# yukw777/EILEV

Measured on AMD Instinct MI355X. Metric: clips/sec (8-frame, 16 in-context) encode+generate, eilev-blip2-opt-2.7b, higher is better.
Workload: dtype bf16

## Files before the change

### eilev_amd/csrc/gemm_pp4.h

```cpp
#pragma once
#include "gemm_common.h"

namespace {

#ifndef EILEV_PP4_DEEP
#define EILEV_PP4_DEEP 1
#endif
template <int EPI, bool F8 = false, int LN = 0, int M16K = 0, bool A3 = false>
__global__ __launch_bounds__(512, 2) void gemm_pp4_kernel(const GemmArgs g) {
    constexpr bool M16 = M16K != 0, HT16 = M16K == 2;
    static_assert(!M16 || !F8, "16 x 16 form: bf16 instances");
    constexpr int BM = 256, BN = 256, NWM = 2, NWN = 4, NW = 8;
    constexpr int WM = BM / NWM, WN = BN / NWN, TM = WM / 32, TN = WN / 32;
    constexpr int STEP = (BM + BN) * 128;
    constexpr int PC = 8;
    static_assert(!A3 || M16, "A3: lean epilogues only");
    constexpr int STG0 = A3 ? 2 * BM * 128 : 2 * STEP;

    extern __shared__ __attribute__((aligned(16))) char smem[];
    auto a_slot = [&](int st) { return smem + (A3 ? (st % 3) * (BM * 128) : (st & 1) * STEP); };
    auto w_slot = [&](int st) { return smem + (A3 ? 3 * (BM * 128) + (st & 1) * (BN * 128) : (st & 1) * STEP + BM * 128); };
    const int tiles_m = (g.M + BM - 1) / BM, tiles_n = (g.N + BN - 1) / BN, ntiles = tiles_m * tiles_n;
    const int tid = threadIdx.x, lane = tid & 63;
    const int wid = __builtin_amdgcn_readfirstlane(tid >> 6);
// ... 169 lines not shown
            for (int i = 0; i < 4; ++i)
#pragma unroll
                for (int j = 0; j < 4; ++j)
                    acc16[i][j] = __builtin_amdgcn_mfma_f32_16x16x32_bf16(bfr[j >> 1][j & 1], af[0][i], acc16[i][j], 0, 0, 0);
        } else {
#pragma unroll
            for (int k2 = 0; k2 < 2; ++k2)
#pragma unroll
                for (int i = 0; i < 2; ++i)
#pragma unroll
                    for (int j = 0; j < 2; ++j)
                        acc[i][j] = __builtin_amdgcn_mfma_f32_32x32x16_bf16(bfr[k2][j], af[k2][i], acc[i][j], 0, 0, 0);
        }
        __builtin_amdgcn_s_setprio(0);
    };
    char *const stg = smem + STG0 + wid * 4096;
    const unsigned stg_sw = (unsigned)(STG0 + wid * 4096 + l31 * 128 + hi * 8) ^ (unsigned)((l31 & 7) << 4);
    const unsigned stg_sw16 = (unsigned)(STG0 + wid * 4096 + l15 * 128 + (g4 & 1) * 8) ^ (unsigned)((((g4 >> 1) ^ (l15 & 7)) << 4));
    const int srow = lane >> 3, schunk = lane & 7;
    auto is_lean = [&](int n0_) {
        return !(n0_ + 128 >= g.N && !(g.dbg & DBG_GEMM_NO_HALF_TILES)) && n0_ + BN <= g.N && !g.out_f32 && g.patch_group == 0 && g.scale_cols == 0 && !g.wscale && !g.ascale &&
               !(g.dbg & (DBG_GEMM_NO_EPILOGUE | DBG_GEMM_NO_STORES | DBG_GEMM_ROW0_STORES)) && !(g.dbg & DBG_GEMM_PP4_NO_PRESTAGE);
    };
    float ln_rs[LN == 1 ? (M16 ? TM16 : TM) : 1];
    auto lean_epilogue = [&](int cm0, int cn0, auto res_c, auto ht_c) {
        constexpr bool RES = decltype(res_c)::value;
        constexpr bool HTE = decltype(ht_c)::value;
        constexpr int NU = HTE ? 2 : TM;
        const int roff = HTE ? hm * 64 : wm * WM, coff = HTE ? hn * 64 : wn * WN;
        if constexpr (M16K == 1) {
            if (cn0 + coff >= g.N) return;
        }
        constexpr bool LNC = LN == 1 && !RES, LNP = LN == 2 && RES;
        typedef __attribute__((ext_vector_type(4))) unsigned u32x4_t;
        const int r0 = cm0 + roff;
        const int rows = g.M - r0 < 0 ? 0 : (g.M - r0 < NU * 32 ? g.M - r0 : NU * 32);
        auto uniform_rsrc = [&](const void *ptr, int bytes) {
            const uint64_t base = (uint64_t)ptr;
            const uint64_t ub = ((uint64_t)(unsigned)__builtin_amdgcn_readfirstlane((int)(base >> 32)) << 32) |
                                (unsigned)__builtin_amdgcn_readfirstlane((int)(unsigned)base);
            return __builtin_amdgcn_make_buffer_rsrc((void *)ub, 0, __builtin_amdgcn_readfirstlane(bytes), 0x00020000);
        };
        const __amdgpu_buffer_rsrc_t rc = uniform_rsrc(reinterpret_cast<bf16 *>(g.C) + (int64_t)r0 * g.ldc + cn0 + coff, rows * (int)(g.ldc * 2));
        const __amdgpu_buffer_rsrc_t rr = uniform_rsrc(RES ? g.resid + (int64_t)r0 * g.ldr + cn0 + coff : g.A, RES ? rows * (int)(g.ldr * 2) : 0);
        const unsigned st_voff = (unsigned)srow * (unsigned)(g.ldc * 2) + schunk * 16, rs_voff = (unsigned)srow * (unsigned)(g.ldr * 2) + schunk * 16;
#ifndef EILEV_HM_AUX
#define EILEV_HM_AUX EILEV_ST_AUX
#endif
        constexpr bool HMI = LN == 1 && !RES && EPI == 0 && M16K == 1;
        const bool hm = HMI && g.hm_tok != 0;
        __amdgpu_buffer_rsrc_t rch = rc;
        unsigned hm_off = 0, hm_off_w = 0;
        int hm_str2 = 0, hm_t = 0;
        if constexpr (HMI) {
            if (hm) {
                const int TOK = g.hm_tok, HD = g.hm_hd, NH = g.hm_heads, D3 = g.N / 3;
                const int n0 = cn0 + coff;
                const int plane = __builtin_amdgcn_readfirstlane(n0 / D3), rr = n0 - plane * D3;
                int2 ent;
                if (rr < NH * 64) {
                    ent.x = (plane * NH + (rr >> 6)) * TOK * HD + schunk * 8;
                    ent.y = 64;
                } else {
                    const int cph = (HD - 64) >> 3, jb = ((rr - NH * 64) >> 3) + schunk, hh = jb / cph;
                    ent.x = (plane * NH + hh) * TOK * HD + TOK * 64 + (jb - hh * cph) * 8;
                    ent.y = HD - 64;
                }
                const int fw = __builtin_amdgcn_readfirstlane(r0 / TOK);
                const int m0 = r0 + srow, f0 = m0 / TOK;
                hm_t = m0 - f0 * TOK;
                hm_str2 = __builtin_amdgcn_readfirstlane(ent.y * 2);
                hm_off = (unsigned)(((f0 - fw) * TOK * g.N + ent.x + hm_t * ent.y) * 2);
                hm_off_w = hm_off + (unsigned)(TOK * g.N * 2) - (unsigned)(TOK * hm_str2);
                const int64_t left = ((int64_t)g.M / TOK - fw) * TOK * g.N * 2;
                rch = uniform_rsrc(reinterpret_cast<bf16 *>(g.C) + (int64_t)fw * TOK * g.N, (int)(unsigned)(left < 0xfffffff0ll ? left : 0xfffffff0ll));
            }
        }
        u32x4_t rv[4];
        auto res_load = [&](int u) {
#pragma unroll
            for (int it = 0; it < 4; ++it) rv[it] = __builtin_amdgcn_raw_buffer_load_b128(rr, rs_voff, (u * 32 + it * 8) * (int)(g.ldr * 2), 0);
        };
        if constexpr (RES) res_load(0);
        bf16x4 biasr[M16 ? 1 : TN][4];
        bf16x4 biasr16[M16 ? TN16 : 1];
        if constexpr (M16) {
#pragma unroll
            for (int j = 0; j < TN16; ++j) {
                if (g.bias) biasr16[j] = *reinterpret_cast<const bf16x4 *>(g.bias + cn0 + coff + j * 16 + g4 * 4);
                else biasr16[j] = (bf16x4){(bf16)0.f, (bf16)0.f, (bf16)0.f, (bf16)0.f};
            }
        } else {
#pragma unroll
        for (int j = 0; j < TN; ++j)
#pragma unroll
            for (int q = 0; q < 4; ++q) {
                if (g.bias) biasr[j][q] = *reinterpret_cast<const bf16x4 *>(g.bias + cn0 + wn * WN + j * 32 + q * 8 + hi * 4);
                else biasr[j][q] = (bf16x4){(bf16)0.f, (bf16)0.f, (bf16)0.f, (bf16)0.f};
            }
        }
        typedef __attribute__((ext_vector_type(2))) float f32x2_t;
        __amdgpu_buffer_rsrc_t rst = rr;
        if constexpr (LNP) rst = uniform_rsrc(g.stat_out + ((int64_t)((cn0 + coff) >> 6) * g.stat_ld + r0) * 2, rows * 8);
        static_for<NU>([&](auto u_c) {
            constexpr int U = decltype(u_c)::value;
            float st1 = 0.0f, st2 = 0.0f;
            bf16x4 rcell[M16 ? 2 : TN][4];
            if constexpr (RES) {
#pragma unroll
                for (int it = 0; it < 4; ++it) {
                    const int row = it * 8 + srow;
                    *reinterpret_cast<u32x4_t *>(stg + row * 128 + ((schunk ^ (row & 7)) << 4)) = rv[it];
                }
                if constexpr (U + 1 < NU) res_load(U + 1);
                if constexpr (M16) {
#pragma unroll
                    for (int ib = 0; ib < 2; ++ib)
#pragma unroll
                        for (int j = 0; j < TN16; ++j) {
                            unsigned ca;
                            asm volatile("v_xor_b32 %0, %1, %2" : "=v"(ca) : "n"(((j * 2) << 4) | (ib << 11)), "v"(stg_sw16));
                            rcell[ib][j] = *reinterpret_cast<const bf16x4 *>(smem + ca);
                        }
                } else {
#pragma unroll
                for (int j = 0; j < TN; ++j)
#pragma unroll
                    for (int q = 0; q < 4; ++q) {
                        unsigned ca;
                        asm volatile("v_xor_b32 %0, %1, %2" : "=v"(ca) : "n"((j * 4 + q) << 4), "v"(stg_sw));
                        rcell[j][q] = *reinterpret_cast<const bf16x4 *>(smem + ca);
                    }
                }
            }
            float st16[2][2] = {{0.0f, 0.0f}, {0.0f, 0.0f}};
            if constexpr (M16) {
#pragma unroll
                for (int ib = 0; ib < 2; ++ib)
#pragma unroll
                    for (int j = 0; j < TN16; ++j) {
                        float v[4];
                        if constexpr (LNC) {
#pragma unroll
                            for (int e = 0; e < 4; ++e) v[e] = fmaf(acc16[2 * U + ib][j][e], ln_rs[2 * U + ib], (float)biasr16[j][e]);
                        } else {
#pragma unroll
                            for (int e = 0; e < 4; ++e) v[e] = acc16[2 * U + ib][j][e] + (float)biasr16[j][e];
                        }
                        if constexpr (LN == 0 && EPI == 0 && !RES) {
                            if (cn0 + coff + j * 16 < g.scale_cols) {
#pragma unroll
                                for (int e = 0; e < 4; ++e) v[e] *= g.scale;
                            }
                        }
                        if constexpr (EPI == 2) {
#pragma unroll
                            for (int e = 0; e < 4; ++e) v[e] = fmaxf(v[e], 0.0f);
                        }
                        if constexpr (EPI == 1) gelu_erf_n<4>(v);
                        if constexpr (RES) {
#pragma unroll
                            for (int e = 0; e < 4; ++e) v[e] += (float)rcell[ib][j][e];
                        }
                        if constexpr (LNP) {
#pragma unroll
                            for (int e = 0; e < 4; ++e) {
                                st16[ib][0] += v[e];
                                st16[ib][1] = fmaf(v[e], v[e], st16[ib][1]);
                            }
                        }
                        unsigned ca;
                        asm volatile("v_xor_b32 %0, %1, %2" : "=v"(ca) : "n"(((j * 2) << 4) | (ib << 11)), "v"(stg_sw16));
                        *reinterpret_cast<bf16x4 *>(smem + ca) = (bf16x4){(bf16)v[0], (bf16)v[1], (bf16)v[2], (bf16)v[3]};
                    }
            } else {
#pragma unroll
            for (int j = 0; j < TN; ++j)
#pragma unroll
                for (int q = 0; q < 4; ++q) {
                    float v[4];
                    if constexpr (LNC) {
#pragma unroll
                        for (int e = 0; e < 4; ++e) v[e] = fmaf(acc[U][j][q * 4 + e], ln_rs[U], (float)biasr[j][q][e]);
                    } else {
#pragma unroll
                        for (int e = 0; e < 4; ++e) v[e] = acc[U][j][q * 4 + e] + (float)biasr[j][q][e];
                    }
                    if constexpr (EPI == 2) {
#pragma unroll
                        for (int e = 0; e < 4; ++e) v[e] = fmaxf(v[e], 0.0f);
                    }
                    if constexpr (EPI == 1) gelu_erf_n<4>(v);
                    if constexpr (RES) {
#pragma unroll
                        for (int e = 0; e < 4; ++e) v[e] += (float)rcell[j][q][e];
                    }
                    if constexpr (LNP) {
#pragma unroll
                        for (int e = 0; e < 4; ++e) {
                            st1 += v[e];
                            st2 = fmaf(v[e], v[e], st2);
                        }
                    }
                    unsigned ca;
                    asm volatile("v_xor_b32 %0, %1, %2" : "=v"(ca) : "n"((j * 4 + q) << 4), "v"(stg_sw));
                    *reinterpret_cast<bf16x4 *>(smem + ca) = (bf16x4){(bf16)v[0], (bf16)v[1], (bf16)v[2], (bf16)v[3]};
                }
            }
            if constexpr (LNP && M16) {
                typedef __attribute__((ext_vector_type(2))) unsigned u32x2_t;
#pragma unroll
                for (int ib = 0; ib < 2; ++ib) {
                    float a1 = st16[ib][0], a2 = st16[ib][1];
                    a1 += __shfl_xor(a1, 16); a2 += __shfl_xor(a2, 16);
                    a1 += __shfl_xor(a1, 32); a2 += __shfl_xor(a2, 32);
                    const f32x2_t t = (f32x2_t){a1, a2};
                    if (g4 == 0) __builtin_amdgcn_raw_buffer_store_b64(__builtin_bit_cast(u32x2_t, t), rst, (U * 32 + ib * 16 + l15) * 8, 0, 0);
                }
            } else if constexpr (LNP) {
                typedef __attribute__((ext_vector_type(2))) unsigned u32x2_t;
                const f32x2_t t = (f32x2_t){st1 + __shfl_xor(st1, 32), st2 + __shfl_xor(st2, 32)};
                if (hi == 0) __builtin_amdgcn_raw_buffer_store_b64(__builtin_bit_cast(u32x2_t, t), rst, (U * 32 + l31) * 8, 0, 0);
            }
            __builtin_amdgcn_sched_barrier(0);
            bf16x8 erb[2];
#pragma unroll
            for (int h2 = 0; h2 < 2; ++h2) {
#pragma unroll
                for (int b = 0; b < 2; ++b) {
                    const int row = (h2 * 2 + b) * 8 + srow;
                    erb[b] = *reinterpret_cast<const bf16x8 *>(stg + row * 128 + ((schunk ^ (row & 7)) << 4));
                }
                if (hm) {
                    if constexpr (HMI) {
#pragma unroll
                        for (int b = 0; b < 2; ++b) {
                            const int RO = U * 32 + (h2 * 2 + b) * 8;
                            const unsigned vo = hm_t + RO >= g.hm_tok ? hm_off_w : hm_off;
                            __builtin_amdgcn_raw_buffer_store_b128(__builtin_bit_cast(u32x4_t, erb[b]), rch, vo, RO * hm_str2, EILEV_HM_AUX);
                        }
                    }
                } else {
#pragma unroll
                for (int b = 0; b < 2; ++b)
                    __builtin_amdgcn_raw_buffer_store_b128(__builtin_bit_cast(u32x4_t, erb[b]), rc, st_voff, (U * 32 + (h2 * 2 + b) * 8) * (int)(g.ldc * 2), EILEV_ST_AUX);
                }
            }
            asm volatile("s_nop 1" ::: "memory");
            __builtin_amdgcn_sched_barrier(0);
        });
    };
#define PP_WAIT_LGKM0() __builtin_amdgcn_s_waitcnt(0xC07F)
// ... 266 lines not shown
```

### eilev_amd/csrc/attention.hip

```cpp
#include <type_traits>

#include "common.h"
#include <type_traits>
#include <utility>

int g_attn_force_v1 = 0, g_attn_dbg = 0;
#ifdef EILEV_PROBES
extern "C" int eilev_debug_attn_v1(int on) { g_attn_force_v1 = on & 1; g_attn_dbg = on >> 1; return 0; }
#endif

namespace {

template <int DP, bool DROP = false>
__global__ __launch_bounds__(256) void attn_prefill_kernel(const AttnArgs a) {
    constexpr int KD = DP / 32;
    constexpr int DT = DP / 16;
    constexpr int CH = DP / 8;
    constexpr int KSTR = DP * 2 + 16;
    constexpr int VSTR = 64 * 2 + 16;
    __shared__ __attribute__((aligned(16))) char ks_[64 * KSTR];
    __shared__ __attribute__((aligned(16))) char vt_[DP * VSTR];
    __shared__ int msk_[64];

    const int tid = threadIdx.x, lane = tid & 63, wid = tid >> 6;
// ... 301 lines not shown
        for (int kb = 0; kb < NB; ++kb)
#pragma unroll
            for (int r = 0; r < 16; ++r) {
                const float p = __builtin_amdgcn_exp2f(fmaf(st[kb][r], sl2, nm));
                st[kb][r] = p;
                rs += p;
            }
        rs += __shfl_xor(rs, 32, 64);
        l_run += rs;
        const int v_gb = 2 * (g16 & 1) + ((i16 & 3) >> 1), v_x0 = 2 * (g16 >> 1) + (i16 >> 3);
        const char *vrow = vt_ + (toff + 4 * (g16 >> 1) + (i16 >> 2)) * RS;
        const char *vbase = SWZ ? vrow + ((v_gb ^ v_x0) << 4) + 8 * (i16 & 1) : vrow + (16 * (g16 & 1) + (i16 & 3) * 4) * 2;
#pragma unroll
        for (int kb = 0; kb < NB; ++kb) {
#pragma unroll
            for (int s2 = 0; s2 < 2; ++s2) {
                bf16x8 pb;
#pragma unroll
                for (int j = 0; j < 8; ++j) pb[j] = (bf16)st[kb][8 * s2 + j];
#pragma unroll
                for (int db = 0; db < DB; ++db) {
                    const char *va = vbase + (kb * 32 + 16 * s2) * RS + (SWZ ? 0 : db * 64);
                    const bf16x4 lo = __builtin_amdgcn_ds_read_tr16_b64_v4bf16((lds_bf16x4_t *)(va + (SWZ ? db * 64 : 0)));
                    const bf16x4 hi4 = __builtin_amdgcn_ds_read_tr16_b64_v4bf16((lds_bf16x4_t *)(va + 8 * RS + (SWZ ? (db ^ 1) * 64 : 0)));
                    const bf16x8 vf = {lo[0], lo[1], lo[2], lo[3], hi4[0], hi4[1], hi4[2], hi4[3]};
                    o[db] = __builtin_amdgcn_mfma_f32_32x32x16_bf16(vf, pb, o[db], 0, 0, 0);
                }
            }
        }
    };

    for (int t = 0; t < ntiles; ++t) {
        const int cur = t & 1;
        if (t + 1 < ntiles && !(a.dbg & DBG_ATTN_NO_PREFETCH)) stage_in(cur ^ 1, t + 1);
        if (active && !(a.dbg & DBG_ATTN_NO_COMPUTE)) {
            const int kv0 = t * 64;
            int vis_end = kv_end;
            if (a.causal) vis_end = min(vis_end, min(a.sq - 1, q0 + 31) + off + 1);
            const bool plain = msk[128 + cur] != 0 && (!a.causal || kv0 + 63 <= q0 + off);
            using two = std::integral_constant<int, 2>;
            using one = std::integral_constant<int, 1>;
            if (NWQ > 8 || (DB == 4 && NWQ == 8)) {
                if (kv0 < vis_end) {
                    if (plain) tile_body(one{}, std::false_type{}, cur, kv0);
                    else tile_body(one{}, std::true_type{}, cur, kv0);
                }
                if (kv0 + 32 < vis_end) {
                    if (plain) tile_body(one{}, std::false_type{}, cur, kv0 + 32);
                    else tile_body(one{}, std::true_type{}, cur, kv0 + 32);
                }
            } else if (kv0 + 32 < vis_end) {
                if (plain) tile_body(two{}, std::false_type{}, cur, kv0);
                else tile_body(two{}, std::true_type{}, cur, kv0);
            } else if (kv0 < vis_end) {
                tile_body(one{}, std::true_type{}, cur, kv0);
            }
        }
        asm volatile("s_waitcnt vmcnt(0)" ::: "memory");
        __syncthreads();
    }

    {
        constexpr int OS = DB == 4 ? 272 : 200;
        char *reg = smem + wid * (32 * OS);
        const float inv = l_run > 0.0f ? 1.0f / l_run : 0.0f;
#pragma unroll
// ... 272 lines not shown
                stage(a.k + (int64_t)bn * a.k_bs + (int64_t)hn * a.k_hs, cur ^ 1);
            }
            pv_phase(pr, l, ob, 0);
            if (more) load_q(pn, 0, qf[0]);
            FA_TS(6);
            if constexpr (TWO) {
                s_phase(kaddr, qf[1], sc);
                FA_TS(7);
                l = softmax(sc, pr);
                FA_TS(8);
                pv_phase(pr, l, ob, 1);
                if (more) load_q(pn, 1, qf[1]);
                FA_TS(9);
            }
        }
    };
    if (two_tiles) run(std::true_type{});
    else run(std::false_type{});
#undef FA_TS
#undef FA_BARRIER
}

template <int HD, int NT>
int launch_attn_frame(const AttnArgs &a, hipStream_t s) {
    constexpr int CH = HD / 8;
    constexpr int NPIECE = (NT * 16 * CH + (12 - CH) + 63) / 64;
    constexpr int smem = 3 * NPIECE * 1024;
    const int npairs = a.batch * a.heads;
    const int grid = npairs < eilev_grid_cus() ? npairs : eilev_grid_cus();
    return eilev_launch<attn_frame_kernel<HD, NT>>(dim3(grid), dim3(576), smem, s, a);
}

#include "attn_frame3.h"

template <int NWQ, int DB = 3, bool REL = false>
int launch_attn_v2(const AttnArgs &a, hipStream_t s) {
    size_t smem = attn_v2_rel_offset(NWQ, a.hd) + (REL ? (size_t)(a.rel_n + 2 * ATTN_V2_REL_SLACK) * sizeof(float) : 0);
    const dim3 grid((a.sq + 32 * NWQ - 1) / (32 * NWQ), a.heads, a.batch), block(64 * NWQ);
    return eilev_launch<attn_prefill_v2_kernel<NWQ, DB, REL>>(grid, block, smem, s, a);
}

}

int launch_attention(const AttnArgs &a_in, hipStream_t s) {
    AttnArgs a = a_in;
    a.dbg = g_attn_dbg;
    if (a.batch <= 0 || a.sq <= 0) return EILEV_OK;
    if (!a.q || !a.k || !a.v || !a.o || a.skv <= 0) return EILEV_E_BADARG;
    if ((a.hd & 7) || a.hd > 128 || (a.ldq & 7) || (a.ldk & 7) || (a.ldv & 7) || (a.ldo & 7) || ((uintptr_t)a.o & 15) || (a.q_hs & 7) ||
        (a.k_hs & 7) || (a.v_hs & 7) || (a.o_hs & 7) || (a.q_bs & 7) || (a.k_bs & 7) || (a.v_bs & 7) || (a.o_bs & 7))
        return EILEV_E_UNSUPPORTED;
    if (a.hm) {
        if (a.hd != 88 || a.sq != 257 || a.skv != 257 || a.causal || a.key_mask || a.rel_tab || a.drop_thr || (a.q_hs & 7) || (a.q_bs & 7) ||
            a.q_hs != a.k_hs || a.q_hs != a.v_hs || (int64_t)a.sq * a.hd * 2 >= 0x7fff0000ll)
            return EILEV_E_UNSUPPORTED;
        return launch_attn_frame3<88, 17, true>(a, s);
    }
    if (!g_attn_force_v1 && !(a.dbg & DBG_ATTN_NO_FRAME) && !a.rel_tab && !a.drop_thr && a.hd == 88 && a.sq == a.skv && a.sq > 256 && a.sq <= 272 && !a.causal && !a.key_mask &&
        a.ldk == a.ldv && !(a.ldq & 3) && (int64_t)a.sq * a.ldk * 2 < 0x7fff0000ll) {
#ifdef EILEV_PROBES
        if (a.dbg & DBG_ATTN_HEAD_MAJOR) {
            a.ldq = a.ldk = a.ldv = a.hd;
            a.q_hs = a.k_hs = a.v_hs = (int64_t)a.sq * a.hd;
            a.k = a.q + (int64_t)a.sq * a.heads * a.hd;
            a.v = a.q + 2 * (int64_t)a.sq * a.heads * a.hd;
        }
#endif
        if (a.sq == 257 && !(a.dbg & DBG_ATTN_NO_FRAME3) && ((a.dbg & (DBG_ATTN_FRAME3 | DBG_ATTN_FRAME3_STAMPS)) || a.batch >= 512)) return launch_attn_frame3<88, 17>(a, s);
        return launch_attn_frame<88, 17>(a, s);
    }
    if (!g_attn_force_v1 && !a.drop_thr && a.hd == 64 && a.sq >= 128 && a.skv >= 64 && a.scale > 0.0f &&
        (!a.rel_tab || (a.rel_n <= ATTN_V2_REL_MAX && a.rel_off >= a.skv - 1 && a.rel_off + a.sq <= a.rel_n))) {
        const int qt = (a.sq + 31) / 32;
        if (a.rel_tab) return qt >= 5 ? launch_attn_v2<8, 2, true>(a, s) : launch_attn_v2<4, 2, true>(a, s);
        return qt >= 5 ? launch_attn_v2<8, 2, false>(a, s) : launch_attn_v2<4, 2, false>(a, s);
    }
    if (!g_attn_force_v1 && !a.rel_tab && !a.drop_thr && a.hd == 128 && a.sq >= 64 && a.skv >= 64) {
        const int qt = (a.sq + 31) / 32;
#ifdef EILEV_PROBES
        if (a.dbg & DBG_ATTN_V2_4WAVES) return launch_attn_v2<4, 4>(a, s);
#endif
        return qt >= 5 ? launch_attn_v2<8, 4>(a, s) : launch_attn_v2<4, 4>(a, s);
    }
    if (!g_attn_force_v1 && !a.rel_tab && !a.drop_thr && (a.hd == 80 || a.hd == 88 || a.hd == 72) && a.skv >= 32) {
        const int qt = (a.sq + 31) / 32;
        if (qt == 9 || qt > 16) return (qt == 9) ? launch_attn_v2<9>(a, s) : launch_attn_v2<8>(a, s);
        if (qt >= 5) return launch_attn_v2<8>(a, s);
        if (qt >= 3) return launch_attn_v2<4>(a, s);
        return launch_attn_v2<2>(a, s);
    }
    const dim3 grid((a.sq + 63) / 64, a.heads, a.batch), block(256);
    if (a.drop_thr) {
        if (a.hd <= 64) hipLaunchKernelGGL((attn_prefill_kernel<64, true>), grid, block, 0, s, a);
        else if (a.hd <= 96) hipLaunchKernelGGL((attn_prefill_kernel<96, true>), grid, block, 0, s, a);
        else hipLaunchKernelGGL((attn_prefill_kernel<128, true>), grid, block, 0, s, a);
    } else if (a.hd <= 64) hipLaunchKernelGGL(attn_prefill_kernel<64>, grid, block, 0, s, a);
    else if (a.hd <= 96) hipLaunchKernelGGL(attn_prefill_kernel<96>, grid, block, 0, s, a);
    else hipLaunchKernelGGL(attn_prefill_kernel<128>, grid, block, 0, s, a);
    EILEV_LAUNCH_CHECK();
    return EILEV_OK;
}
```

### eilev_amd/csrc/build.py

```python
from __future__ import annotations

import os
import subprocess
import sys
from concurrent.futures import ThreadPoolExecutor

HERE = os.path.dirname(os.path.abspath(__file__))
SOURCES = ["gemm.hip", "gemm_pp4_ext.hip", "norm.hip", "attention.hip", "misc.hip", "attn_decode.hip", "vision.hip", "opt.hip", "t5.hip", "blocks.hip", "backward.hip", "comm.hip", "gemv.hip"]
HEADERS = ["common.h", "stages.h", "gemm_common.h", "gemm_tiled.h", "gemm_pp4.h", "gemm_w6.h", "gemm_skinny.h", "attn_frame3.h", os.path.join("..", "..", "include", "eilev.h")]
FLAGS = ["--offload-arch=gfx950", "-O3", "-std=c++17", "-fPIC", "-Wall", "-Wno-unused-function",
         "-Wno-pass-failed"]
LIB = os.path.join(HERE, "libeilev_hip.so")
PLD_SOURCE = "pld.hip"
PLD_HEADERS = ["common.h", os.path.join("..", "..", "include", "eilev.h"), os.path.join("..", "..", "include", "eilev_pld.h")]
PLD_LIB = os.path.join(HERE, "libeilev_hip_pld.so")
SAMPLE_SOURCE = "sample.hip"
SAMPLE_HEADERS = ["common.h", os.path.join("..", "..", "include", "eilev.h"), os.path.join("..", "..", "include", "eilev_sample.h")]
SAMPLE_LIB = os.path.join(HERE, "libeilev_hip_sample.so")
RULES_SOURCE = "rules.hip"
RULES_HEADERS = ["common.h", os.path.join("..", "..", "include", "eilev.h"), os.path.join("..", "..", "include", "eilev_rules.h")]
RULES_LIB = os.path.join(HERE, "libeilev_hip_rules.so")


def _hipcc() -> str:
    for c in (os.environ.get("HIPCC"), "/opt/rocm/bin/hipcc", "hipcc"):
        if c and (os.path.sep not in c or os.path.exists(c)):
            return c
    return "hipcc"


def _stale(target: str, deps) -> bool:
    if not os.path.exists(target):
        return True
    t = os.path.getmtime(target)
    return any(os.path.getmtime(d) > t for d in deps)


def build_hip(force: bool = False, verbose: bool = False, variant: str = "", extra_flags=()) -> str:
    hdrs = [os.path.join(HERE, h) for h in HEADERS]
    objdir = os.path.join(HERE, "build", variant) if variant else os.path.join(HERE, "build")
    lib = os.path.join(HERE, f"libeilev_hip_{variant}.so") if variant else LIB
    os.makedirs(objdir, exist_ok=True)
# ... 48 lines not shown
```

### eilev_amd/csrc/common.h

```cpp
#pragma once
#include <hip/hip_runtime.h>
#include <stdint.h>

#include <type_traits>

#include "../../include/eilev.h"

typedef __bf16 bf16;
typedef __attribute__((ext_vector_type(8))) __bf16 bf16x8;
typedef __attribute__((ext_vector_type(4))) __bf16 bf16x4;
typedef __attribute__((ext_vector_type(2))) __bf16 bf16x2;
typedef __attribute__((ext_vector_type(4))) float f32x4;
typedef __attribute__((ext_vector_type(16))) float f32x16;

#define EILEV_HIP_CHECK(expr)                          \
    do {                                               \
        hipError_t _e = (expr);                        \
        if (_e != hipSuccess) return (int)_e;          \
    } while (0)

static inline int eilev_num_cu() {
    static int n = 0;
    if (!n) {
        int dev = 0, cu = 0;
// ... 312 lines not shown
                        int64_t *fin_seq, float *fin_score, int64_t *fin_len, uint8_t *finished, uint8_t *can_improve, int64_t *tokens, int32_t *anc,
                        int gen_cap, int64_t *scratch, hipStream_t s);
int launch_t5_rel_table(const bf16 *rel_w, float *tab, int n, int off, int heads, int bidirectional, int num_buckets, int max_dist,
                        hipStream_t s, const int32_t *state = nullptr);
int launch_gated_gelu(const bf16 *ab, int64_t ld, bf16 *out, int64_t rows, int F, hipStream_t s);
int launch_rows_to_cache(const bf16 *src, int64_t ld, int col0, bf16 *plane, int batch, int rows_per_b, int heads, int hd, int cap,
                         int slot0, hipStream_t s, const int32_t *state = nullptr);
int launch_layernorm(const bf16 *x, int64_t ldx, const bf16 *g, const bf16 *b, bf16 *y, int64_t ldy, int64_t rows,
                     int cols, float eps, hipStream_t s);
int launch_fold_layernorm(const bf16 *w, const bf16 *gamma, const bf16 *beta, const bf16 *bias, int N, int K, bf16 *wf, float *csum, bf16 *bf,
                          hipStream_t s);
int launch_reduce_ln(const float *part, int ks, int mr, int M, int N, const float *wscale, const bf16 *bias, const bf16 *resid, int64_t ldr, bf16 *C,
                     int64_t ldc, const bf16 *gamma, const bf16 *beta, bf16 *ln_out, float eps, hipStream_t s, int ln_frag = 0);
int launch_ln_finalize(const float *part, int slots, int64_t rows, int cols, float eps, float *out, hipStream_t s);

struct AttnArgs {
    const bf16 *q, *k, *v;
    bf16 *o;
    int64_t q_bs, k_bs, v_bs, o_bs;
    int64_t q_hs, k_hs, v_hs, o_hs;
    int64_t ldq, ldk, ldv, ldo;
    int batch, heads, sq, skv, hd;
    float scale;
    int causal;
    const int32_t *key_mask;
    int64_t mask_ld;
    int dbg = 0;
    const float *rel_tab = nullptr;
    int64_t rel_hs = 0;
    int rel_off = 0, rel_n = 0;
    int hm = 0;
    uint32_t drop_thr = 0, drop_seed = 0;
    float drop_scale = 1.0f;
};
static inline AttnArgs attn_rows(const bf16 *q, int64_t ldq, const bf16 *k, int64_t ldk, const bf16 *v, int64_t ldv, bf16 *o, int64_t batch,
                                 int64_t heads, int64_t sq, int64_t skv, int64_t hd, float scale) {
    AttnArgs a;
    a.q = q; a.k = k; a.v = v; a.o = o;
    a.q_bs = sq * ldq; a.k_bs = skv * ldk; a.v_bs = skv * ldv; a.o_bs = sq * heads * hd;
    a.q_hs = a.k_hs = a.v_hs = a.o_hs = hd;
    a.ldq = ldq; a.ldk = ldk; a.ldv = ldv; a.ldo = heads * hd;
    a.batch = (int)batch; a.heads = (int)heads; a.sq = (int)sq; a.skv = (int)skv; a.hd = (int)hd; a.scale = scale; a.causal = 0;
    a.key_mask = nullptr; a.mask_ld = 0;
    return a;
}
static inline AttnArgs attn_cache(const bf16 *q, int64_t ldq, const bf16 *kplane, const bf16 *vplane, int64_t cap, bf16 *o, int64_t batch,
                                  int64_t heads, int64_t sq, int64_t skv, int64_t hd, float scale) {
    AttnArgs a = attn_rows(q, ldq, kplane, hd, vplane, hd, o, batch, heads, sq, skv, hd, scale);
    a.k_bs = a.v_bs = heads * cap * hd;
    a.k_hs = a.v_hs = cap * hd;
    return a;
}
int launch_attention(const AttnArgs &a, hipStream_t s);

struct DecodeAttnArgs {
    const bf16 *qkv = nullptr;
    int64_t ldq = 0;
    const bf16 *kc = nullptr, *vc = nullptr;
    bf16 *out = nullptr;
    const int32_t *attn_mask = nullptr;
    const int32_t *state = nullptr;
    int batch = 0, seq_len = 0, cap = 0, heads = 0, hd = 0;
    float *part = nullptr; size_t part_bytes = 0;
    int fuse_new = 0;
    const float *rel_tab = nullptr;
    int64_t rel_hs = 0; int rel_off = 0;
    bf16 *kg = nullptr, *vg = nullptr;
// ... 17 lines not shown
```

### eilev_amd/csrc/opt.hip

```cpp
#include "stages.h"

namespace {
inline int64_t opt_ws_rows(int64_t M) { return (M > 16 && M < 32) ? 32 : M; }

struct OptBufs {
    bf16 *h, *x, *att, *qkv, *ffn;
    int32_t *pid;
    float *scratch;
    uint8_t *a8;
    float *a8_scale;
    size_t used;
};

OptBufs carve_opt(const EilevDims *d, int64_t M, void *ws) {
    Carver cv{(char *)ws};
    OptBufs b;
    M = opt_ws_rows(M);
    b.h = cv.take<bf16>((size_t)M * d->t_hidden);
    b.x = cv.take<bf16>((size_t)M * d->t_hidden);
    b.att = cv.take<bf16>((size_t)M * d->t_hidden);
    b.qkv = cv.take<bf16>((size_t)M * 3 * d->t_hidden);
    b.ffn = cv.take<bf16>((size_t)M * d->t_ffn);
    b.pid = cv.take<int32_t>((size_t)M);
    b.scratch = cv.take<float>(kSkinnyScratch / sizeof(float));
// ... 201 lines not shown
        }
        return opt_rows_head(d, w, b, M, logits, s);
    }
    const int D = d->t_hidden;
    for (int l = 0; l < d->t_layers; ++l) {
        const EilevOptLayer *L = &w->layers[l];
        DecodeAttnArgs al = at_block(a, l, kv_layer, gen_layer);
        al.out_frag = frag;
        if (l == 0) RC(launch_layernorm(b.h, D, (const bf16 *)L->ln1_w, (const bf16 *)L->ln1_b, b.x, D, M, D, d->t_eps, s));
        RC(opt_qkv(d, w, l, b, M, s, l > 0 ? frag : 0));
        RC(launch_attn_decode(al, s));
        const bool last = l + 1 == d->t_layers;
        RC(opt_tail(d, w, l, b, M, s, last ? w->final_ln_w : w->layers[l + 1].ln1_w, last ? w->final_ln_b : w->layers[l + 1].ln1_b, frag));
    }
    GemmArgs g = opt_lm_head(d, w, b, M, logits);
    g.a_frag = frag;
    return launch_gemm(g, 5, s);
}

int opt_blocks(const EilevDims *d, const EilevOptWeights *w, const OptBufs &b, const void *inputs_embeds, const int32_t *attn_mask, int64_t batch,
               int64_t rows, int64_t past_len, bool from_cache, void *kv_cache, int64_t kv_capacity, void *hidden, hipStream_t s) {
    const int D = d->t_hidden, H = d->t_heads, hd = D / H;
    const int64_t M = batch * rows, total = past_len + rows;
    RC(launch_pos_embed((const bf16 *)inputs_embeds, (const bf16 *)w->embed_positions, attn_mask, b.pid, b.h, (int)batch, (int)total, D,
                        s, (int)past_len));
    const KvCache kv(batch, D, kv_capacity);
    const size_t hs_bytes = (size_t)M * D * sizeof(bf16);
    for (int l = 0; l < d->t_layers; ++l) {
        const EilevOptLayer *L = &w->layers[l];
        bf16 *kc = kv.k((bf16 *)kv_cache, l), *vc = kv.v((bf16 *)kv_cache, l);
        if (hidden) RC(copy_hidden(hidden, l, b.h, hs_bytes, s));
        RC(launch_layernorm(b.h, D, (const bf16 *)L->ln1_w, (const bf16 *)L->ln1_b, b.x, D, M, D, d->t_eps, s));
        RC(opt_qkv(d, w, l, b, M, s));
        RC(launch_kv_write(b.qkv, kc, vc, (int)batch, (int)rows, H, hd, (int)kv_capacity, (int)total, nullptr, s, (int)past_len));
        AttnArgs a = from_cache ? attn_cache(b.qkv, 3 * D, kc, vc, kv_capacity, b.att, batch, H, rows, total, hd, 1.0f)
                                : attn_rows(b.qkv, 3 * D, b.qkv + D, 3 * D, b.qkv + 2 * D, 3 * D, b.att, batch, H, rows, total, hd, 1.0f);
        a.causal = 1; a.key_mask = attn_mask; a.mask_ld = total;
        RC(launch_attention(a, s));
        RC(opt_tail(d, w, l, b, M, s));
    }
    RC(launch_layernorm(b.h, D, (const bf16 *)w->final_ln_w, (const bf16 *)w->final_ln_b, b.x, D, M, D, d->t_eps, s));
    if (hidden) RC(copy_hidden(hidden, d->t_layers, b.x, hs_bytes, s));
    return EILEV_OK;
}

int opt_prefill_impl(const EilevDims *d, const EilevOptWeights *w, const void *inputs_embeds, const int32_t *attn_mask, int64_t batch,
                     int64_t seq_len, void *kv_cache, int64_t kv_capacity, float *logits_last, float *logits_all, void *hidden,
                     void *workspace, size_t workspace_bytes, void *stream) {
    if (!d || !w || !inputs_embeds || !attn_mask || !kv_cache || !workspace || batch <= 0 || seq_len <= 0) return EILEV_E_BADARG;
    if (seq_len > kv_capacity || seq_len > d->max_pos) return EILEV_E_BADARG;
    if (!dims_ok_opt(d)) return EILEV_E_UNSUPPORTED;
    if (workspace_bytes < eilev_opt_workspace_bytes(d, batch, seq_len)) return EILEV_E_WORKSPACE;
    hipStream_t s = (hipStream_t)stream;
    const int D = d->t_hidden;
    const int64_t M = batch * seq_len;
    const OptBufs b = carve_opt(d, M, workspace);
    RC(opt_blocks(d, w, b, inputs_embeds, attn_mask, batch, seq_len, 0, false, kv_cache, kv_capacity, hidden, s));
    if (logits_all) {
        GemmArgs g = mk_gemm(b.x, D, w->embed_tokens, D, nullptr, nullptr, 0, logits_all, d->vocab, M, d->vocab, D, 0);
        g.out_f32 = 1;
        RC(launch_gemm(g, 5, s));
    }
    if (logits_last) {
        GemmArgs g = sk_gemm(b.scratch, b.x + (seq_len - 1) * (int64_t)D, seq_len * (int64_t)D, w->embed_tokens, D, nullptr, nullptr, 0,
                             logits_last, d->vocab, batch, d->vocab, D, 0);
        g.out_f32 = 1;
        RC(launch_gemm(g, 5, s));
    }
    return EILEV_OK;
}
// ... 157 lines not shown
```

Measured before the change: 223.8.

## Add row-side lean epilogue for 16x16 residual+LN-stat GEMM path

For the 16x16 MFMA residual-plus-LayerNorm-stats epilogue, the accumulators are now transposed through LDS as fp32 so each lane holds 8 contiguous columns of a row. Bias, residual add, bf16 pack and the per-row sum and sum-of-squares are then done row-wise, with DPP row reductions replacing cross-lane shuffles. Residual prefetch is interleaved with the stores. The change also adds a compile-time probe macro that can zero the store or residual buffer ranges for epilogue cost experiments; it defaults off. The cost is extra fp32 LDS traffic and a new code path whose swizzle and stat layout must match what the downstream LayerNorm consumer expects.

```diff
diff --git a/eilev_amd/csrc/gemm_pp4.h b/eilev_amd/csrc/gemm_pp4.h
--- a/eilev_amd/csrc/gemm_pp4.h
+++ b/eilev_amd/csrc/gemm_pp4.h
@@ -225,6 +225,7 @@
             if (cn0 + coff >= g.N) return;
         }
         constexpr bool LNC = LN == 1 && !RES, LNP = LN == 2 && RES;
+        constexpr bool ROWSIDE = M16 && LNP;
         typedef __attribute__((ext_vector_type(4))) unsigned u32x4_t;
         const int r0 = cm0 + roff;
         const int rows = g.M - r0 < 0 ? 0 : (g.M - r0 < NU * 32 ? g.M - r0 : NU * 32);
@@ -234,8 +235,11 @@
                                 (unsigned)__builtin_amdgcn_readfirstlane((int)(unsigned)base);
             return __builtin_amdgcn_make_buffer_rsrc((void *)ub, 0, __builtin_amdgcn_readfirstlane(bytes), 0x00020000);
         };
-        const __amdgpu_buffer_rsrc_t rc = uniform_rsrc(reinterpret_cast<bf16 *>(g.C) + (int64_t)r0 * g.ldc + cn0 + coff, rows * (int)(g.ldc * 2));
-        const __amdgpu_buffer_rsrc_t rr = uniform_rsrc(RES ? g.resid + (int64_t)r0 * g.ldr + cn0 + coff : g.A, RES ? rows * (int)(g.ldr * 2) : 0);
+        #ifndef EILEV_PP4_PROBE_EPI
+#define EILEV_PP4_PROBE_EPI 0
+#endif
+        const __amdgpu_buffer_rsrc_t rc = uniform_rsrc(reinterpret_cast<bf16 *>(g.C) + (int64_t)r0 * g.ldc + cn0 + coff, (EILEV_PP4_PROBE_EPI & 2) ? 0 : rows * (int)(g.ldc * 2));
+        const __amdgpu_buffer_rsrc_t rr = uniform_rsrc(RES ? g.resid + (int64_t)r0 * g.ldr + cn0 + coff : g.A, RES && !(EILEV_PP4_PROBE_EPI & 1) ? rows * (int)(g.ldr * 2) : 0);
         const unsigned st_voff = (unsigned)srow * (unsigned)(g.ldc * 2) + schunk * 16, rs_voff = (unsigned)srow * (unsigned)(g.ldr * 2) + schunk * 16;
 #ifndef EILEV_HM_AUX
 #define EILEV_HM_AUX EILEV_ST_AUX
@@ -277,7 +281,8 @@
         if constexpr (RES) res_load(0);
         bf16x4 biasr[M16 ? 1 : TN][4];
         bf16x4 biasr16[M16 ? TN16 : 1];
-        if constexpr (M16) {
+        if constexpr (ROWSIDE) {
+        } else if constexpr (M16) {
 #pragma unroll
             for (int j = 0; j < TN16; ++j) {
                 if (g.bias) biasr16[j] = *reinterpret_cast<const bf16x4 *>(g.bias + cn0 + coff + j * 16 + g4 * 4);
@@ -294,7 +299,69 @@
         }
         typedef __attribute__((ext_vector_type(2))) float f32x2_t;
         __amdgpu_buffer_rsrc_t rst = rr;
-        if constexpr (LNP) rst = uniform_rsrc(g.stat_out + ((int64_t)((cn0 + coff) >> 6) * g.stat_ld + r0) * 2, rows * 8);
+        if constexpr (LNP) rst = uniform_rsrc(g.stat_out + ((int64_t)((cn0 + coff) >> 6) * g.stat_ld + r0) * 2, (EILEV_PP4_PROBE_EPI & 2) ? 0 : rows * 8);
+        if constexpr (ROWSIDE) {
+            float biasf[8];
+#pragma unroll
+            for (int h = 0; h < 2; ++h) {
+                bf16x4 b4 = (bf16x4){(bf16)0.f, (bf16)0.f, (bf16)0.f, (bf16)0.f};
+                if (g.bias) b4 = *reinterpret_cast<const bf16x4 *>(g.bias + cn0 + coff + schunk * 8 + h * 4);
+#pragma unroll
+                for (int e = 0; e < 4; ++e) biasf[h * 4 + e] = (float)b4[e];
+            }
+            const unsigned wa = (unsigned)(l15 * 256 + ((g4 ^ l15) << 4));
+            const unsigned ra = (unsigned)(srow * 256 + (((2 * schunk) ^ srow) << 4));
+            const unsigned stat_voff = schunk == 0 ? (unsigned)srow * 8u : 0x80000000u;
+            auto row_sum8 = [](float x) {
+                x += __builtin_bit_cast(float, __builtin_amdgcn_update_dpp(0, __builtin_bit_cast(int, x), 0xB1, 0xf, 0xf, true));
+                x += __builtin_bit_cast(float, __builtin_amdgcn_update_dpp(0, __builtin_bit_cast(int, x), 0x4E, 0xf, 0xf, true));
+                x += __builtin_bit_cast(float, __builtin_amdgcn_update_dpp(0, __builtin_bit_cast(int, x), 0x141, 0xf, 0xf, true));
+                return x;
+            };
+            static_for<NU>([&](auto u_c) {
+                constexpr int U = decltype(u_c)::value;
+                typedef __attribute__((ext_vector_type(2))) unsigned u32x2_t;
+#pragma unroll
+                for (int ib = 0; ib < 2; ++ib) {
+#pragma unroll
+                    for (int j = 0; j < TN16; ++j) *reinterpret_cast<f32x4_t *>(stg + (wa ^ (unsigned)(j << 6))) = acc16[2 * U + ib][j];
+                    bf16x8 ob[2];
+                    f32x2_t stt[2];
+#pragma unroll
+                    for (int p = 0; p < 2; ++p) {
+                        const int it = ib * 2 + p;
+                        const unsigned rp = (ra ^ (unsigned)(p << 7)) + p * 2048;
+                        const f32x4_t s0 = *reinterpret_cast<const f32x4_t *>(stg + rp), s1 = *reinterpret_cast<const f32x4_t *>(stg + (rp ^ 16u));
+                        const bf16x8 rb = __builtin_bit_cast(bf16x8, rv[it]);
+                        float v[8];
+#pragma unroll
+                        for (int e = 0; e < 4; ++e) {
+                            v[e] = (s0[e] + biasf[e]) + (float)rb[e];
+                            v[4 + e] = (s1[e] + biasf[4 + e]) + (float)rb[4 + e];
+                        }
+                        if constexpr (U + 1 < NU) rv[it] = __builtin_amdgcn_raw_buffer_load_b128(rr, rs_voff, ((U + 1) * 32 + it * 8) * (int)(g.ldr * 2), 0);
+                        float a1 = 0.0f, a2 = 0.0f;
+#pragma unroll
+                        for (int e = 0; e < 8; ++e) {
+                            a1 += v[e];
+                            a2 = fmaf(v[e], v[e], a2);
+                        }
+                        stt[p] = (f32x2_t){row_sum8(a1), row_sum8(a2)};
+                        ob[p] = (bf16x8){(bf16)v[0], (bf16)v[1], (bf16)v[2], (bf16)v[3], (bf16)v[4], (bf16)v[5], (bf16)v[6], (bf16)v[7]};
+                    }
+                    __builtin_amdgcn_sched_barrier(0);
+#pragma unroll
+                    for (int p = 0; p < 2; ++p)
+                        __builtin_amdgcn_raw_buffer_store_b128(__builtin_bit_cast(u32x4_t, ob[p]), rc, st_voff, (U * 32 + (ib * 2 + p) * 8) * (int)(g.ldc * 2), EILEV_ST_AUX);
+                    asm volatile("s_nop 1" ::: "memory");
+                    __builtin_amdgcn_sched_barrier(0);
+#pragma unroll
+                    for (int p = 0; p < 2; ++p)
+                        __builtin_amdgcn_raw_buffer_store_b64(__builtin_bit_cast(u32x2_t, stt[p]), rst, stat_voff, (U * 32 + (ib * 2 + p) * 8) * 8, 0);
+                }
+            });
+            return;
+        }
         static_for<NU>([&](auto u_c) {
             constexpr int U = decltype(u_c)::value;
             float st1 = 0.0f, st2 = 0.0f;
@@ -326,7 +393,6 @@
                     }
                 }
             }
-            float st16[2][2] = {{0.0f, 0.0f}, {0.0f, 0.0f}};
             if constexpr (M16) {
 #pragma unroll
                 for (int ib = 0; ib < 2; ++ib)
@@ -355,13 +421,6 @@
 #pragma unroll
                             for (int e = 0; e < 4; ++e) v[e] += (float)rcell[ib][j][e];
                         }
-                        if constexpr (LNP) {
-#pragma unroll
-                            for (int e = 0; e < 4; ++e) {
-                                st16[ib][0] += v[e];
-                                st16[ib][1] = fmaf(v[e], v[e], st16[ib][1]);
-                            }
-                        }
                         unsigned ca;
                         asm volatile("v_xor_b32 %0, %1, %2" : "=v"(ca) : "n"(((j * 2) << 4) | (ib << 11)), "v"(stg_sw16));
                         *reinterpret_cast<bf16x4 *>(smem + ca) = (bf16x4){(bf16)v[0], (bf16)v[1], (bf16)v[2], (bf16)v[3]};
@@ -400,17 +459,7 @@
                     *reinterpret_cast<bf16x4 *>(smem + ca) = (bf16x4){(bf16)v[0], (bf16)v[1], (bf16)v[2], (bf16)v[3]};
                 }
             }
-            if constexpr (LNP && M16) {
-                typedef __attribute__((ext_vector_type(2))) unsigned u32x2_t;
-#pragma unroll
-                for (int ib = 0; ib < 2; ++ib) {
-                    float a1 = st16[ib][0], a2 = st16[ib][1];
-                    a1 += __shfl_xor(a1, 16); a2 += __shfl_xor(a2, 16);
-                    a1 += __shfl_xor(a1, 32); a2 += __shfl_xor(a2, 32);
-                    const f32x2_t t = (f32x2_t){a1, a2};
-                    if (g4 == 0) __builtin_amdgcn_raw_buffer_store_b64(__builtin_bit_cast(u32x2_t, t), rst, (U * 32 + ib * 16 + l15) * 8, 0, 0);
-                }
-            } else if constexpr (LNP) {
+            if constexpr (LNP) {
                 typedef __attribute__((ext_vector_type(2))) unsigned u32x2_t;
                 const f32x2_t t = (f32x2_t){st1 + __shfl_xor(st1, 32), st2 + __shfl_xor(st2, 32)};
                 if (hi == 0) __builtin_amdgcn_raw_buffer_store_b64(__builtin_bit_cast(u32x2_t, t), rst, (U * 32 + l31) * 8, 0, 0);
```

Measured after the change: 224.4 (median of 6 runs). About the same (+0.3%).

## Fuse OPT prefill KV-cache write into attention and add split-KV cross-attention kernel

Applied to the files above, without the earlier changes.

The OPT prefill attention kernel (head dim 72/80/88, causal, sq==skv) now copies each staged K/V tile from LDS straight into the KV cache, so the separate kv_write launch can be skipped when no hidden-state capture is requested. A new cross-attention kernel handles the short-query, long-KV case (hd 64, sq<=64, skv>=512, unmasked). It spreads KV blocks across 8 waves, each running its own online softmax, then merges the partial results through LDS. This aims to cut a launch and a global round-trip per layer, and to raise parallelism for the short-query attention. The cost is extra global stores inside the attention loop and a new LDS merge path.

```diff
diff --git a/eilev_amd/csrc/attention.hip b/eilev_amd/csrc/attention.hip
--- a/eilev_amd/csrc/attention.hip
+++ b/eilev_amd/csrc/attention.hip
@@ -357,6 +357,19 @@
 
     for (int t = 0; t < ntiles; ++t) {
         const int cur = t & 1;
+        if constexpr (DB == 3) {
+            if (a.cache_k && (t * 64) / (32 * NWQ) == (int)blockIdx.x) {
+                const int nch = min(64, a.skv - t * 64) * CHS;
+                const char *img = smem + cur * 2 * T;
+                const int64_t at = ((((int64_t)b * a.heads + h) * a.cache_cap + a.cache_slot0) + t * 64) * a.hd;
+                int p0 = tid;
+                asm volatile("" : "+v"(p0));
+                for (int p = p0; p < nch; p += 64 * NWQ) {
+                    *reinterpret_cast<bf16x8 *>(a.cache_k + at + p * 8) = *reinterpret_cast<const bf16x8 *>(img + p * 16);
+                    *reinterpret_cast<bf16x8 *>(a.cache_v + at + p * 8) = *reinterpret_cast<const bf16x8 *>(img + T + p * 16);
+                }
+            }
+        }
         if (t + 1 < ntiles && !(a.dbg & DBG_ATTN_NO_PREFETCH)) stage_in(cur ^ 1, t + 1);
         if (active && !(a.dbg & DBG_ATTN_NO_COMPUTE)) {
             const int kv0 = t * 64;
@@ -695,6 +708,7 @@
 }
 
 #include "attn_frame3.h"
+#include "attn_cross.h"
 
 template <int NWQ, int DB = 3, bool REL = false>
 int launch_attn_v2(const AttnArgs &a, hipStream_t s) {
@@ -738,6 +752,9 @@
         if (a.rel_tab) return qt >= 5 ? launch_attn_v2<8, 2, true>(a, s) : launch_attn_v2<4, 2, true>(a, s);
         return qt >= 5 ? launch_attn_v2<8, 2, false>(a, s) : launch_attn_v2<4, 2, false>(a, s);
     }
+    if (!g_attn_force_v1 && !a.rel_tab && !a.drop_thr && !a.causal && !a.key_mask && a.hd == 64 && a.sq <= 64 && a.skv >= 512 && a.scale > 0.0f &&
+        !(((uintptr_t)a.q | (uintptr_t)a.k | (uintptr_t)a.v) & 15))
+        return launch_attn_cross<8>(a, s);
     if (!g_attn_force_v1 && !a.rel_tab && !a.drop_thr && a.hd == 128 && a.sq >= 64 && a.skv >= 64) {
         const int qt = (a.sq + 31) / 32;
 #ifdef EILEV_PROBES
@@ -745,6 +762,9 @@
 #endif
         return qt >= 5 ? launch_attn_v2<8, 4>(a, s) : launch_attn_v2<4, 4>(a, s);
     }
+    if (a.cache_k && (g_attn_force_v1 || !attn_writes_cache(a) || !a.cache_v || a.cache_slot0 < 0 || a.cache_slot0 + a.skv > a.cache_cap ||
+                      (((uintptr_t)a.cache_k | (uintptr_t)a.cache_v) & 15)))
+        return EILEV_E_UNSUPPORTED;
     if (!g_attn_force_v1 && !a.rel_tab && !a.drop_thr && (a.hd == 80 || a.hd == 88 || a.hd == 72) && a.skv >= 32) {
         const int qt = (a.sq + 31) / 32;
         if (qt == 9 || qt > 16) return (qt == 9) ? launch_attn_v2<9>(a, s) : launch_attn_v2<8>(a, s);
diff --git a/eilev_amd/csrc/attn_cross.h b/eilev_amd/csrc/attn_cross.h
--- /dev/null
+++ b/eilev_amd/csrc/attn_cross.h
@@ -0,0 +1,154 @@
+constexpr int ATTN_CROSS_VRS = 144;
+constexpr int ATTN_CROSS_PS = 68;
+template <int NW>
+constexpr int attn_cross_smem() {
+    return NW * 32 * ATTN_CROSS_PS * 4 + NW * 2 * 32 * 4;
+}
+
+template <int NW>
+__global__ __launch_bounds__(64 * NW) void attn_cross_kernel(const AttnArgs a) {
+    constexpr int VRS = ATTN_CROSS_VRS, PS = ATTN_CROSS_PS;
+    static_assert(NW * 32 * VRS <= NW * 32 * PS * 4, "the V regions overlay the merge image");
+    extern __shared__ __attribute__((aligned(16))) char smem[];
+    const int tid = threadIdx.x, lane = tid & 63;
+    const int wid = __builtin_amdgcn_readfirstlane(tid >> 6);
+    const int l31 = lane & 31, hi = lane >> 5, g16 = lane >> 4, i16 = lane & 15;
+    const int b = blockIdx.z, h = blockIdx.y, q0 = blockIdx.x * 32;
+    const int qrow = q0 + l31;
+    const float sl2 = a.scale * 1.44269504088896340736f;
+    const bf16 *qp = a.q + (int64_t)b * a.q_bs + (int64_t)h * a.q_hs;
+    const bf16 *kp = a.k + (int64_t)b * a.k_bs + (int64_t)h * a.k_hs;
+    const bf16 *vp = a.v + (int64_t)b * a.v_bs + (int64_t)h * a.v_hs;
+    const int nblk = (a.skv + 31) >> 5;
+
+    bf16x8 qf[4], kr[4], vr[4];
+#pragma unroll
+    for (int kd = 0; kd < 4; ++kd)
+        qf[kd] = qrow < a.sq ? *reinterpret_cast<const bf16x8 *>(qp + (int64_t)qrow * a.ldq + hi * 32 + kd * 8) : zero8();
+    auto load_kv = [&](int blk) {
+        const int kv0 = blk * 32;
+        const bf16 *krow = kp + (int64_t)min(kv0 + l31, a.skv - 1) * a.ldk + hi * 32;
+#pragma unroll
+        for (int kd = 0; kd < 4; ++kd) kr[kd] = *reinterpret_cast<const bf16x8 *>(krow + kd * 8);
+#pragma unroll
+        for (int i = 0; i < 4; ++i) {
+            const int p = i * 64 + lane;
+            vr[i] = *reinterpret_cast<const bf16x8 *>(vp + (int64_t)min(kv0 + (p >> 3), a.skv - 1) * a.ldv + (p & 7) * 8);
+        }
+    };
+
+    float m_run = -1e30f, l_run = 0.0f;
+    f32x16 o[2];
+#pragma unroll
+    for (int i = 0; i < 2; ++i)
+#pragma unroll
+        for (int r = 0; r < 16; ++r) o[i][r] = 0.0f;
+    char *vst = smem + wid * (32 * VRS);
+    const char *vbase = vst + (4 * hi + (i16 >> 2)) * VRS + (16 * (g16 & 1) + (i16 & 3) * 4) * 2;
+
+    int blk = wid;
+    if (blk < nblk) load_kv(blk);
+    for (; blk < nblk; blk += NW) {
+        const int kv0 = blk * 32;
+#pragma unroll
+        for (int i = 0; i < 4; ++i) {
+            const int p = i * 64 + lane;
+            *reinterpret_cast<bf16x8 *>(vst + (p >> 3) * VRS + (p & 7) * 16) = vr[i];
+        }
+        f32x16 st;
+#pragma unroll
+        for (int r = 0; r < 16; ++r) st[r] = 0.0f;
+#pragma unroll
+        for (int kd = 0; kd < 4; ++kd) st = __builtin_amdgcn_mfma_f32_32x32x16_bf16(kr[kd], qf[kd], st, 0, 0, 0);
+        if (blk + NW < nblk) load_kv(blk + NW);
+        if (kv0 + 32 > a.skv) {
+#pragma unroll
+            for (int r = 0; r < 16; ++r) st[r] = kv0 + (r & 3) + 8 * (r >> 2) + 4 * hi < a.skv ? st[r] : -1e30f;
+        }
+        float mx = st[0];
+#pragma unroll
+        for (int r = 1; r < 16; ++r) mx = fmaxf(mx, st[r]);
+        mx = fmaxf(mx, __shfl_xor(mx, 32, 64));
+        const float m_new = fmaxf(m_run, mx * sl2);
+        const float alpha = __builtin_amdgcn_exp2f(m_run - m_new);
+        m_run = m_new;
+        float rs = 0.0f;
+#pragma unroll
+        for (int r = 0; r < 16; ++r) {
+            const float p = __builtin_amdgcn_exp2f(fmaf(st[r], sl2, -m_new));
+            st[r] = p;
+            rs += p;
+        }
+        rs += __shfl_xor(rs, 32, 64);
+        l_run = l_run * alpha + rs;
+#pragma unroll
+        for (int i = 0; i < 2; ++i)
+#pragma unroll
+            for (int r = 0; r < 16; ++r) o[i][r] *= alpha;
+        __builtin_amdgcn_wave_barrier();
+#pragma unroll
+        for (int s2 = 0; s2 < 2; ++s2) {
+            bf16x8 pb;
+#pragma unroll
+            for (int j = 0; j < 8; ++j) pb[j] = (bf16)st[8 * s2 + j];
+#pragma unroll
+            for (int db = 0; db < 2; ++db) {
+                const char *va = vbase + 16 * s2 * VRS + db * 64;
+                const bf16x4 lo = __builtin_amdgcn_ds_read_tr16_b64_v4bf16((lds_bf16x4_t *)va);
+                const bf16x4 hi4 = __builtin_amdgcn_ds_read_tr16_b64_v4bf16((lds_bf16x4_t *)(va + 8 * VRS));
+                const bf16x8 vf = {lo[0], lo[1], lo[2], lo[3], hi4[0], hi4[1], hi4[2], hi4[3]};
+                o[db] = __builtin_amdgcn_mfma_f32_32x32x16_bf16(vf, pb, o[db], 0, 0, 0);
+            }
+        }
+        __builtin_amdgcn_wave_barrier();
+    }
+
+    float *part = reinterpret_cast<float *>(smem);
+    float *ml = part + NW * 32 * PS;
+    if (hi == 0) {
+        ml[(wid * 2 + 0) * 32 + l31] = m_run;
+        ml[(wid * 2 + 1) * 32 + l31] = l_run;
+    }
+    __syncthreads();
+    {
+        float mall = -1e30f;
+#pragma unroll
+        for (int w = 0; w < NW; ++w) mall = fmaxf(mall, ml[(w * 2) * 32 + l31]);
+        const float f = __builtin_amdgcn_exp2f(m_run - mall);
+        float *pr = part + (wid * 32 + l31) * PS;
+#pragma unroll
+        for (int db = 0; db < 2; ++db)
+#pragma unroll
+            for (int g = 0; g < 4; ++g) {
+                const f32x4 w4 = {o[db][g * 4] * f, o[db][g * 4 + 1] * f, o[db][g * 4 + 2] * f, o[db][g * 4 + 3] * f};
+                *reinterpret_cast<f32x4 *>(pr + db * 32 + g * 8 + hi * 4) = w4;
+            }
+    }
+    __syncthreads();
+    for (int e = tid; e < 32 * 16; e += 64 * NW) {
+        const int row = e >> 4, d4 = (e & 15) * 4;
+        float mall = -1e30f;
+#pragma unroll
+        for (int w = 0; w < NW; ++w) mall = fmaxf(mall, ml[(w * 2) * 32 + row]);
+        float l = 0.0f;
+        f32x4 acc = {0.f, 0.f, 0.f, 0.f};
+#pragma unroll
+        for (int w = 0; w < NW; ++w) {
+            l += ml[(w * 2 + 1) * 32 + row] * __builtin_amdgcn_exp2f(ml[(w * 2) * 32 + row] - mall);
+            acc += *reinterpret_cast<const f32x4 *>(part + (w * 32 + row) * PS + d4);
+        }
+        if (q0 + row < a.sq) {
+            const float inv = l > 0.0f ? 1.0f / l : 0.0f;
+            bf16x4 w4;
+#pragma unroll
+            for (int r = 0; r < 4; ++r) w4[r] = (bf16)(acc[r] * inv);
+            *reinterpret_cast<bf16x4 *>(a.o + (int64_t)b * a.o_bs + (int64_t)h * a.o_hs + (int64_t)(q0 + row) * a.ldo + d4) = w4;
+        }
+    }
+}
+
+template <int NW>
+int launch_attn_cross(const AttnArgs &a, hipStream_t s) {
+    const dim3 grid((a.sq + 31) / 32, a.heads, a.batch), block(64 * NW);
+    return eilev_launch<attn_cross_kernel<NW>>(grid, block, attn_cross_smem<NW>(), s, a);
+}
diff --git a/eilev_amd/csrc/build.py b/eilev_amd/csrc/build.py
--- a/eilev_amd/csrc/build.py
+++ b/eilev_amd/csrc/build.py
@@ -7,7 +7,7 @@
 
 HERE = os.path.dirname(os.path.abspath(__file__))
 SOURCES = ["gemm.hip", "gemm_pp4_ext.hip", "norm.hip", "attention.hip", "misc.hip", "attn_decode.hip", "vision.hip", "opt.hip", "t5.hip", "blocks.hip", "backward.hip", "comm.hip", "gemv.hip"]
-HEADERS = ["common.h", "stages.h", "gemm_common.h", "gemm_tiled.h", "gemm_pp4.h", "gemm_w6.h", "gemm_skinny.h", "attn_frame3.h", os.path.join("..", "..", "include", "eilev.h")]
+HEADERS = ["common.h", "stages.h", "gemm_common.h", "gemm_tiled.h", "gemm_pp4.h", "gemm_w6.h", "gemm_skinny.h", "attn_frame3.h", "attn_cross.h", os.path.join("..", "..", "include", "eilev.h")]
 FLAGS = ["--offload-arch=gfx950", "-O3", "-std=c++17", "-fPIC", "-Wall", "-Wno-unused-function",
          "-Wno-pass-failed"]
 LIB = os.path.join(HERE, "libeilev_hip.so")
diff --git a/eilev_amd/csrc/common.h b/eilev_amd/csrc/common.h
--- a/eilev_amd/csrc/common.h
+++ b/eilev_amd/csrc/common.h
@@ -368,7 +368,12 @@
     int hm = 0;
     uint32_t drop_thr = 0, drop_seed = 0;
     float drop_scale = 1.0f;
+    bf16 *cache_k = nullptr, *cache_v = nullptr;
+    int cache_cap = 0, cache_slot0 = 0;
 };
+static inline bool attn_writes_cache(const AttnArgs &a) {
+    return (a.hd == 72 || a.hd == 80 || a.hd == 88) && a.causal && a.sq == a.skv && a.skv >= 32 && !a.rel_tab && !a.drop_thr && !a.hm;
+}
 static inline AttnArgs attn_rows(const bf16 *q, int64_t ldq, const bf16 *k, int64_t ldk, const bf16 *v, int64_t ldv, bf16 *o, int64_t batch,
                                  int64_t heads, int64_t sq, int64_t skv, int64_t hd, float scale) {
     AttnArgs a;
diff --git a/eilev_amd/csrc/opt.hip b/eilev_amd/csrc/opt.hip
--- a/eilev_amd/csrc/opt.hip
+++ b/eilev_amd/csrc/opt.hip
@@ -257,10 +257,14 @@
         if (hidden) RC(copy_hidden(hidden, l, b.h, hs_bytes, s));
         RC(launch_layernorm(b.h, D, (const bf16 *)L->ln1_w, (const bf16 *)L->ln1_b, b.x, D, M, D, d->t_eps, s));
         RC(opt_qkv(d, w, l, b, M, s));
-        RC(launch_kv_write(b.qkv, kc, vc, (int)batch, (int)rows, H, hd, (int)kv_capacity, (int)total, nullptr, s, (int)past_len));
         AttnArgs a = from_cache ? attn_cache(b.qkv, 3 * D, kc, vc, kv_capacity, b.att, batch, H, rows, total, hd, 1.0f)
                                 : attn_rows(b.qkv, 3 * D, b.qkv + D, 3 * D, b.qkv + 2 * D, 3 * D, b.att, batch, H, rows, total, hd, 1.0f);
         a.causal = 1; a.key_mask = attn_mask; a.mask_ld = total;
+        if (!from_cache && !hidden && attn_writes_cache(a)) {
+            a.cache_k = kc; a.cache_v = vc; a.cache_cap = (int)kv_capacity; a.cache_slot0 = 0;
+        } else {
+            RC(launch_kv_write(b.qkv, kc, vc, (int)batch, (int)rows, H, hd, (int)kv_capacity, (int)total, nullptr, s, (int)past_len));
+        }
         RC(launch_attention(a, s));
         RC(opt_tail(d, w, l, b, M, s));
     }
```

New measurement: 222.5 before, 223.1 after, median of 6. About the same (+0.3%).
